# url-kaist/Quatro

Measured on AMD Instinct MI355X. Metric: scan-pair registrations/sec (KITTI 64-ch, ~5k corr) + rot/trans err vs ref, higher is better.
Workload: dtype f32 (voxel grid, FPFH, 33-D matching: f16-split MFMA filter, exact f32 decision) / f64 (consistency graph, GNC-TLS, COTE); 1 GPU; composite: qtr_register_pair_corr per step on a synthetic KITTI-64-shaped scan pair (voxel 0.3 m), back end on 5000 planted correspondences, one pair at a time, inputs resident in HBM (--full: the detailed description)

## Files before the change

quatro_amd/csrc/capi.hip:

```cpp
#include <dlfcn.h>

#include <algorithm>
#include <atomic>
#include <memory>
#include <mutex>
#include <new>
#include <thread>
#include <vector>

#include "common.h"
#include "frontend.h"
#include "solver.h"
#include "stage_times.h"

struct RcclIdByValue {
  char internal[QTR_COMM_ID_BYTES];
};

struct Slot {
  hipStream_t stream = nullptr;
  hipStream_t stream2 = nullptr;
  hipEvent_t ev[EV_COUNT] = {};
  hipEvent_t ev_vox = nullptr;
  hipStream_t stream3 = nullptr;
// ... 108 lines not shown
  int spin_wait = 1;
  bool pre_on = false;
  qtr_pw_params pre_pw;
  qtr_ip_params pre_ip;
  std::atomic<bool> long_lists{false};
  struct Callers {
    std::atomic<int> live{0};
  };
  std::shared_ptr<Callers> callers = std::make_shared<Callers>();
  std::mutex share_mu;
  int share_val = 1, share_gen = 0;
  std::atomic<int> gen_inflight[4] = {};
  unsigned long long uid = 0;
  int stage_events = 1;
  int corr_overlap = 1;
  int nn_event_stride = 1;
  int icp_block = 0;
  std::mutex kf_mu;
  std::vector<qtr_keyframe*> keyframes;
  std::vector<qtr_place_index*> place_indexes;
  std::vector<qtr_voxel_map*> voxel_maps;
  char err[512];
};

static std::atomic<unsigned long long> g_handle_uid{0};
static void vmap_free_all(qtr_handle* h);

#define QTR_TRY(expr)                  \
  do {                                 \
    const int rc_ = (expr);            \
// ... 368 lines not shown
  if (!out) return QTR_ERR_BAD_ARG;
  *out = nullptr;
  qtr_handle* h = new (std::nothrow) qtr_handle();
  if (!h) return QTR_ERR_CAPACITY;
  h->err[0] = 0;
  h->device = device;
  h->uid = g_handle_uid.fetch_add(1, std::memory_order_relaxed) + 1;
  {
    const char* hw = getenv("QTR_HOST_WAIT");
    h->spin_wait = (hw && strcmp(hw, "block") == 0) ? 0 : 1;
    const char* se = getenv("QTR_STAGE_EVENTS");
    h->stage_events = (se && atoi(se) == 0) ? 0 : 1;
    h->nn_event_stride = h->stage_events ? 1 : 0;
    const char* co = getenv("QTR_CORR_OVERLAP");
    h->corr_overlap = (co && atoi(co) == 0) ? 0 : 1;
    const char* ib = getenv("QTR_ICP_BLOCK");
    h->icp_block = ib ? std::max(0, atoi(ib)) : 0;
  }
  if (limits)
    h->lim = *limits;
  else
    qtr_default_limits(&h->lim);
  if (h->lim.max_points < 64 || h->lim.max_voxels < 64 || h->lim.max_corr < 64 || h->lim.n_slots < 1 ||
      h->lim.max_corr > 32768 || h->lim.max_voxels > h->lim.max_points || h->lim.max_long_neighbors < 0 ||
      h->lim.max_voxels > QTR_NN_MAX_ROWS) {
    delete h;
    return QTR_ERR_BAD_ARG;
  }
  if (h->lim.max_long_neighbors == 0)
    h->lim.max_long_neighbors = (int)std::min<long long>(128LL * h->lim.max_voxels, 1LL << 30);
// ... 1057 lines not shown
  int prio_least = 0, prio_greatest = 0;
  QTR_HIP_TRY(h, hipDeviceGetStreamPriorityRange(&prio_least, &prio_greatest));
  if (!s.ev_fork) QTR_HIP_TRY(h, hipEventCreateWithFlags(&s.ev_fork, hipEventDisableTiming));
  if (!s.ev_join) QTR_HIP_TRY(h, hipEventCreateWithFlags(&s.ev_join, hipEventDisableTiming));
  if (prio_greatest != prio_least) QTR_HIP_TRY(h, hipStreamCreateWithPriority(&s.stream3, hipStreamNonBlocking, prio_least));
  else QTR_HIP_TRY(h, hipStreamCreateWithFlags(&s.stream3, hipStreamNonBlocking));
  return QTR_OK;
}

struct CorrEarly {
  const float* src = nullptr;
  const float* tgt = nullptr;
  int n = 0, mem = QTR_MEM_HOST;
  const qtr_params* prm = nullptr;
  bool enqueued = false;
  int seq = 0;
  const float4 *cs = nullptr, *ct = nullptr;
  std::unique_ptr<InFlight> in_flight;
};
static int corr_early_enqueue(qtr_handle* h, Slot& s, CorrEarly& ce) {
  ce.enqueued = true;
  const bool ev_on = h->stage_events != 0;
  QTR_HIP_TRY(h, hipStreamWaitEvent(s.stream3, s.ev_fork, 0));
  if (ev_on) QTR_HIP_TRY(h, hipEventRecord(s.ev[EV_BE0], s.stream3));
  QTR_TRY(corr_stage(h, s, ce.src, ce.tgt, ce.n, ce.mem, s.stream3, &ce.cs, &ce.ct));
  s.last_L = ce.n;
  s.last_Wb = (((ce.n + 63) / 64) + 3) & ~3;
  s.sb.mail_seq = ce.seq = ++s.seq;
  ce.in_flight.reset(new InFlight(h));
  QTR_HIP_TRY(h, solver_enqueue(s.sb, ce.cs, ce.ct, ce.n, *ce.prm, s.stream3, ev_on ? s.ev[EV_GRAPH] : nullptr,
                                ev_on ? s.ev[EV_CLIQUE] : nullptr, false, true));
  if (ev_on) QTR_HIP_TRY(h, hipEventRecord(s.ev[EV_SOLVE], s.stream3));
  return QTR_OK;
}

struct CountsText {
  char s[40];
  CountsText(int nc, int a, int b, const char* pair_form = "%d / %d") { snprintf(s, sizeof(s), nc > 1 ? pair_form : "%d", a, b); }
// ... 68 lines not shown
  if (fp->normal_radius > fp->fpfh_radius) {
    snprintf(h->err, sizeof(h->err), "[FPFHManager]: Normal should be lower than fpfh_radius!!!!");
    return QTR_ERR_BAD_ARG;
  }
  if (Ps <= 0 || Pt <= 0 || !src_raw4 || !tgt_raw4) {
    snprintf(h->err, sizeof(h->err), "Invalid or empty point cloud dataset given!");
    return QTR_ERR_BAD_ARG;
  }
  if (Ps > h->lim.max_points || Pt > h->lim.max_points) {
    snprintf(h->err, sizeof(h->err), "cloud exceeds max_points=%d", h->lim.max_points);
    return QTR_ERR_CAPACITY;
  }
  QTR_HIP_TRY(h, hipSetDevice(h->device));
  if (early && !early->enqueued) {
    QTR_TRY(ensure_stream3(h, s));
    QTR_HIP_TRY(h, hipEventRecord(s.ev_fork, s.stream));
  }
  const float4 *d_s = (const float4*)src_raw4, *d_t = (const float4*)tgt_raw4;
  if (mem == QTR_MEM_HOST) {
    QTR_HIP_TRY(h, hipMemcpyAsync(s.in_src, src_raw4, (size_t)Ps * 16, hipMemcpyHostToDevice, s.stream));
    QTR_HIP_TRY(h, hipMemcpyAsync(s.in_tgt, tgt_raw4, (size_t)Pt * 16, hipMemcpyHostToDevice, s.stream));
    d_s = s.in_src;
    d_t = s.in_tgt;
  }
  if (h->stage_events) QTR_HIP_TRY(h, hipEventRecord(s.ev[EV_BEGIN], s.stream));
  const float4* raws[2] = {d_s, d_t};
  const int P2[2] = {Ps, Pt};
  auto beside_voxels = [&]() -> int {
    QTR_HIP_TRY(h, hipEventRecord(s.ev_vox, s.stream));
    const int on_device[2] = {-1, -1};
    QTR_HIP_TRY(h, hipStreamWaitEvent(s.stream2, s.ev_vox, 0));
// ... 70 lines not shown
    struct DrainOnReturn {
      hipStream_t st;
      bool armed = true;
      ~DrainOnReturn() {
        if (armed) (void)hipStreamSynchronize(st);
      }
    } drain{s.stream3};
    if (rc == QTR_OK) rc = wait_mail(h, s, s.stream3, MAIL_SEQ_SOLVE, ce.seq);
    if (rc == QTR_OK) rc = solve_followup(h, s, ce.cs, ce.ct, n_corr, prm, s.stream3, h->stage_events != 0);
    if (rc != QTR_OK) {
      return res->status = rc;
    }
    ce.in_flight.reset();
    result_from_mail(s, res);
    rc = res->status;
    QTR_HIP_TRY(h, hipEventRecord(s.ev_join, s.stream3));
    QTR_HIP_TRY(h, hipStreamWaitEvent(s.stream, s.ev_join, 0));
    if (h->stage_events) QTR_HIP_TRY(h, hipEventRecord(s.ev[EV_END], s.stream));
    rc = finish_registration(h, s, rc, TIMES_PAIR_OVERLAP, res, clique, nullptr, final_inliers, cap, mem_out, s.stream);
    drain.armed = rc != QTR_OK && rc != QTR_ERR_CLIQUE_TOO_SMALL;
    return rc;
  }
  int rc = front_device(h, s, src_raw4, Ps, tgt_raw4, Pt, fp, mem_in, true, &res->n_src, &res->n_tgt, &L, given);
  if (n_matched) *n_matched = L;
  res->n_corr = given ? n_corr : L;
  if (rc != QTR_OK) return res->status = rc;
  const float4 *cs = s.m_src, *ct = s.m_tgt;
  if (given) QTR_TRY(corr_stage(h, s, corr_src, corr_tgt, n_corr, mem_out, s.stream, &cs, &ct));
  rc = solve_device(h, s, cs, ct, res->n_corr, prm, res, true);
  return finish_registration(h, s, rc, TIMES_PAIR, res, clique, nullptr, final_inliers, cap, mem_out, s.stream);
}

// ... 2072 lines not shown
```

quatro_amd/csrc/frontend.h:

```cpp
#pragma once
#include "common.h"
#include "front_verdict.h"

#define QTR_KMAX 256
#define NBIG_LDS_KEYS 8192
#define RADIX_TILE 1024
#define NORM_BINS 192

#define QTR_NN_MAX_ROWS ((1 << 20) - 32)
#define QTR_CELL_CAP (1 << 21)
enum { MC_NCORR = 0, MC_HIDDEN_I = 1, MC_HIDDEN_J = 2, MC_NCROSS = 3, MC_NTUPLE = 4, MC_SWAPPED = 5, MC_NQ0 = 6, MC_NHIT = 7,
       MC_RECHECK0 = 8, MC_RECHECK1 = 9, MC_NSPLIT0 = 10, MC_NSPLIT1 = 11 ,
       MC_UNSAFE = 12,
       MC_TAILERR = 13  };

enum { MAIL_VOX0 = 0, MAIL_VOX1 = 16, MAIL_MATCH = 32, MAIL_CNT0 = 48, MAIL_CNT1 = 64, MAIL_SEQ_VOX0 = 96, MAIL_SEQ_VOX1 = 97,
       MAIL_SEQ_MATCH = 98, MAIL_SEQ_SOLVE = 99, MAIL_SEQ_ICP_BOX = 100, MAIL_SEQ_ICP = 101, MAIL_SOLVER = 128,
       MAIL_ICP_BOX = 256, MAIL_ICP = 272, MAIL_INTS = 512 };

struct CloudBufs {
  int* counts = nullptr;
  u32* mm = nullptr;
  u32* mm_part = nullptr;
  float4* vox = nullptr;
// ... 86 lines not shown
  const float* QT;
  int qt_pad;
  const float* baseTb;
  const int* brow;
  const int* bstart;
  const int* qorder;
  u64* best;
  int nq_slot, rc_slot;
};
struct NnPartial {
  float b1, b2;
  int i1;
  int pad;
};
#define TAIL_MAXWG 256
struct MatchView {
  NnDir d[2];
  const float4 *vox_i, *vox_j;
  const float *mean_i, *mean_j;
  const float *fpfh_i, *fpfh_j;
  float *baseT_i, *queryT_i, *norms_i, *baseT_j, *queryT_j, *norms_j;
  float *baseTb_i, *baseTb_j;
  uint4 *baseH_i, *baseH_j, *queryH_i, *queryH_j, *queryH_c;
  int *nb_row_i, *nb_row_j, *nb_start_i, *nb_start_j;
  u64 *hash_i, *hash_j, *table_i, *table_j;
  int dd_mask;
  int n_large, n_small, pad_large, pad_small, swapped, ns, nt;
  u64 *best_small, *best_large;
  int *nn_of_small, *nn_of_large, *cross_i, *cross_j, *flags, *scan, *passed, *tgt_of_src, *corr, *mcounts;
  NnPartial* partial;
// ... 45 lines not shown
  float* queryT_c = nullptr;
  float* norms_c = nullptr;
  uint4* queryH_c = nullptr;
  int dd_slots = 0;
  int *nc_cnt = nullptr, *nc_fill = nullptr, *nc_off = nullptr, *nc_list = nullptr;
  int* mail = nullptr;
  float4* m_src = nullptr;
  float4* m_tgt = nullptr;
  int m_cap = 0;
  int vox_passes = 4;
  int vox_fewer = 0;
  bool gathered = false;
  int mail_seq = 0;
  int nn_engine = 2;
  int n_cu = 256;
  int nn_events = 1;
  hipEvent_t ev_nn[4] = {};
};

size_t frontend_scratch_bytes(int max_points, int max_voxels);
void frontend_carve(FrontBufs& F, void* base, int max_points, int max_voxels);
hipError_t frontend_init_attributes();

hipError_t voxelize_enqueue(FrontBufs& F, int nc, const float4* const* raw, const int* P, float leaf, hipStream_t st,
                            int passes = 4, float cell_side = 0.f);
hipError_t set_count_enqueue(CloudBufs& C, int which, int value, hipStream_t st);
hipError_t fpfh_enqueue(FrontBufs& F, int first, int nc, const int* n, float r_normal, float r_fpfh, hipStream_t st,
                        bool with_mean, bool origin_known, bool long_lists, bool desc_prep = false,
                        int max_ncell = 0 );
hipError_t mean_enqueue(FrontBufs& F, int first, int nc, const int* n, hipStream_t st, int cap = 0);
// ... 16 lines not shown
```

quatro_amd/csrc/frontend.hip:

```cpp
#include <stdlib.h>

#include <type_traits>
#include <vector>

#include "common.h"
#include "frontend.h"

__device__ __forceinline__ u32 enc_f32(float f) {
  const u32 b = __float_as_uint(f);
  return (b & 0x80000000u) ? ~b : (b | 0x80000000u);
}
__device__ __forceinline__ float dec_f32(u32 e) {
  const u32 b = (e & 0x80000000u) ? (e & 0x7fffffffu) : ~e;
  return __uint_as_float(b);
}


__global__ void k_set_count(int* counts, int which, int value) {
  if (threadIdx.x == 0 && blockIdx.x == 0) counts[which] = value;
}

__device__ __forceinline__ void d_minmax(const float4* __restrict__ pts, int n, u32* __restrict__ part) {
  float mn[3] = {INFINITY, INFINITY, INFINITY}, mx[3] = {-INFINITY, -INFINITY, -INFINITY};
  for (int i = blockIdx.x * blockDim.x + threadIdx.x; i < n; i += gridDim.x * blockDim.x) {
// ... 1706 lines not shown
  while (m < 2 * max_voxels) m <<= 1;
  return m;
}
size_t frontend_scratch_bytes(int max_points, int max_voxels) {
  size_t per_cloud = 0;
  per_cloud += 4096 + MM_MAX_PARTS * 32 + 256;
  per_cloud += (size_t)max_voxels * (16 + 16 + 132 + 132);
  per_cloud += 2 * (size_t)max_points * 8;
  per_cloud += (size_t)(4096 * ((max_points + RADIX_TILE - 1) / RADIX_TILE) + 8192) * 4 + 65536;
  per_cloud += (size_t)((max_points + RADIX_TILE - 1) / RADIX_TILE + 64) * 4 * (RADIX_TILE / VOX_TILE_SINGLE) + 256;
  per_cloud += (size_t)max_voxels * 4 * 2 + 64;
  per_cloud += (size_t)max_voxels * QTR_KMAX * 8;
  per_cloud += (size_t)max_voxels * (16 + 72) + 512;
  per_cloud += 2 * (size_t)(QTR_CELL_CAP + 4096) * 4 + 512;
  per_cloud += (size_t)max_points * 16 + 256;
  size_t shared = (size_t)max_voxels * 64 + 16384 + 2 * TAIL_MAXWG * 4;
  shared += (size_t)max_voxels * (4 + 4 + 4 + 8) + (size_t)max_voxels * 4 * 6 + 4096;
  const size_t vpad = ((size_t)max_voxels + 511) / 512 * 512;
  per_cloud += 3 * 34 * vpad * 4 + (size_t)max_voxels * 8 + 4096;
  per_cloud += 2 * (vpad * 224 + 2 * 7168) + 512;
  per_cloud += (size_t)max_voxels * 8 + (size_t)dedup_slots(max_voxels) * 8 + 512;
  shared += vpad * 32 * 16 + 4 * ((size_t)max_voxels * 4 + 1024);
  shared += (size_t)max_voxels * 4 + 34 * vpad * 4 + vpad * 4 + 1024;
  shared += vpad * 224 + 2 * 7168 + 256 + (size_t)max_voxels * 4 + 1024;
  return 2 * per_cloud + shared + 64 * 256;
}

void frontend_carve(FrontBufs& F, void* base, int max_points, int max_voxels) {
  char* p = (char*)base;
  auto take = [&](size_t bytes) {
    char* r = p;
// ... 34 lines not shown
    C.nb_row = (int*)take((size_t)max_voxels * 4);
    C.nb_start = (int*)take((NORM_BINS + 2) * 4);
    C.norms = (float*)take((size_t)max_voxels * 4);
    C.max_norm = (u32*)take(64);
    C.dd_hash = (u64*)take((size_t)max_voxels * 8);
    C.dd_table = (u64*)take((size_t)dedup_slots(max_voxels) * 8);
  }
  F.dd_slots = dedup_slots(max_voxels);
  F.best_small = (u64*)take((size_t)max_voxels * 8);
  F.best_large = (u64*)take((size_t)max_voxels * 8);
  F.nn_of_small = (int*)take((size_t)max_voxels * 4);
  F.nn_of_large = (int*)take((size_t)max_voxels * 4);
  F.cross_i = (int*)take((size_t)max_voxels * 8);
  F.cross_j = (int*)take((size_t)max_voxels * 8);
  F.flags = (int*)take((size_t)max_voxels * 4);
  F.scan = (int*)take((size_t)max(max_voxels + 1, 2 * TAIL_MAXWG) * 4);
  F.passed = (int*)take((size_t)max_voxels * 8);
  F.tgt_of_src = (int*)take((size_t)max_voxels * 4);
  F.corr = (int*)take((size_t)max_voxels * 16);
  F.nc_cnt = (int*)take((size_t)max_voxels * 4);
  F.nc_fill = (int*)take((size_t)max_voxels * 4);
  F.nc_off = (int*)take((size_t)(max_voxels + 1) * 4);
  F.nc_list = (int*)take((size_t)max_voxels * 8);
  F.mcounts = (int*)take(16 * 4);
  F.nn_partial = take((((size_t)max_voxels + 511) / 512 * 512) * 32 * 16);
  F.recheck_rows = (int*)take((size_t)max_voxels * 4);
  F.recheck_thr = (float*)take((size_t)max_voxels * 4);
  F.recheck_span = (int2*)take((size_t)max_voxels * 8);
  F.hit_rows = (int*)take((size_t)max_voxels * 4);
  F.queryT_c = (float*)take(34 * (((size_t)max_voxels + 511) / 512 * 512) * 4);
  F.norms_c = (float*)take((((size_t)max_voxels + 511) / 512 * 512) * 4);
  F.queryH_c = (uint4*)take((((size_t)max_voxels + 511) / 512 * 512) * 224 + 2 * 7168);
  F.recheck_q = (int*)take((size_t)max_voxels * 4);
  {
    const char* e = QTR_ENGINE_ENV("QTR_NN_ENGINE");
    F.nn_engine = (e && strcmp(e, "exact") == 0) ? 0 : (e && strcmp(e, "mfma32") == 0) ? 1 : 2;
    int dev = 0, cus = 0;
    if (hipGetDevice(&dev) == hipSuccess &&
        hipDeviceGetAttribute(&cus, hipDeviceAttributeMultiprocessorCount, dev) == hipSuccess && cus > 0)
      F.n_cu = cus;
  }
}

hipError_t match_init_attributes();
hipError_t frontend_init_attributes() {
  hipError_t e;
  if ((e = hipFuncSetAttribute((const void*)k2_neighbors_big<false>, hipFuncAttributeMaxDynamicSharedMemorySize,
                               NBIG_LDS_KEYS * 8)) != hipSuccess)
    return e;
  if ((e = hipFuncSetAttribute((const void*)k2_neighbors_big<true>, hipFuncAttributeMaxDynamicSharedMemorySize,
                               NBIG_LDS_KEYS * 8)) != hipSuccess)
// ... 4 lines not shown
```

quatro_amd/csrc/match.hip:

```cpp
#include <vector>

#include "common.h"
#include "frontend.h"

#define NN_TILE 64
#define CROSS_LDS_BYTES (156 * 1024)
#define NN_STRIDE 36

#define LAUNCH_MV_K(kern, K, a, grid, block, lds, st, ...)                                                       \
  do {                                                                                                          \
    if ((a).ext)                                                                                                \
      hipLaunchKernelGGL((kern<true, K>), grid, block, lds, st, (ViewExt<MatchView>{(a).ext, {0, 0, 0}}), (a).one, ##__VA_ARGS__); \
    else                                                                                                        \
      hipLaunchKernelGGL((kern<false, K>), grid, block, lds, st, (ViewExt<MatchView>{nullptr, {0, 0, 0}}), (a).one, ##__VA_ARGS__); \
  } while (0)
#define LAUNCH_MV_EV(kern, a, grid, block, lds, st, e0, e1, ...)                                                 \
  do {                                                                                                          \
    if ((a).ext)                                                                                                \
      hipExtLaunchKernelGGL((kern<true>), grid, block, lds, st, e0, e1, 0, (ViewExt<MatchView>{(a).ext, {0, 0, 0}}), (a).one, ##__VA_ARGS__);  \
    else                                                                                                        \
      hipExtLaunchKernelGGL((kern<false>), grid, block, lds, st, e0, e1, 0, (ViewExt<MatchView>{nullptr, {0, 0, 0}}), (a).one, ##__VA_ARGS__); \
  } while (0)
#define LAUNCH_MV(kern, a, grid, block, lds, st, ...)                                       \
  do {                                                                                      \
// ... 1265 lines not shown
    for (int i = threadIdx.x; i < n_zero; i += blockDim.x) zero_words[i] = 0;
  if (gid < 16) V.mcounts[gid] = (gid == MC_SWAPPED) ? V.swapped : (gid == MC_NQ0) ? V.n_small : 0;
  const int pv = V.tuple ? 0 : 1;
  const int np = V.crosscheck ? V.n_small : V.n_small + V.n_large;
  for (int i = gid; i < np; i += gsz) V.passed[i] = pv;
  if (!V.crosscheck)
    for (int i = gid; i < V.ns; i += gsz) V.nc_cnt[i] = V.nc_fill[i] = 0;
  for (int i = gid; i < V.ns; i += gsz) V.tgt_of_src[i] = -1;
  for (int i = gid; i < V.n_small; i += gsz) V.best_small[i] = ~0ULL;
  for (int i = gid; i < V.n_large; i += gsz) V.best_large[i] = ~0ULL;
  if (clear_tables)
    for (int i = gid; i <= V.dd_mask; i += gsz) {
      V.table_i[i] = ~0ULL;
      V.table_j[i] = ~0ULL;
    }
  for (int i = gid; i < 2 * TAIL_MAXWG; i += gsz) V.scan[i] = 0;
}

template <bool EXT>
__global__ __launch_bounds__(1024) void k_hit_compact(ViewExt<MatchView> x, MatchView one, int bin_order, int nn_X) {
  const MatchView& V = EXT ? x.ext[blockIdx.z] : one;
  extern __shared__ u32 hit_bits[];
  __shared__ int wsum[16];
  const int tid = threadIdx.x, lane = tid & 63, wave = tid >> 6;
  const int n = V.n_large, nw = (n + 31) / 32, ns = V.n_small;
  QTR_STAMP(STAMP_HIT_COMPACT, 0)
  for (int w = tid; w < nw; w += 1024) hit_bits[w] = 0u;
  __syncthreads();
  for (int j0 = tid; j0 < ns; j0 += 16 * 1024) {
    u64 b[16];
#pragma unroll
// ... 99 lines not shown
    V.flags[i] = V.crosscheck ? ((b != ~0ULL && back == i) ? 1 : 0) : ((b != ~0ULL) ? 1 : 0);
  }
}

template <bool EXT>
__global__ __launch_bounds__(1024) void k_scan_flags(ViewExt<MatchView> x, MatchView one) {
  const MatchView& V = EXT ? x.ext[blockIdx.z] : one;
  d_block_scan(V.flags, V.scan, V.n_large, [](int x) { return x; });
}
template <bool EXT>
__global__ __launch_bounds__(1024) void k_scan_nonneg(ViewExt<MatchView> x, MatchView one) {
  const MatchView& V = EXT ? x.ext[blockIdx.z] : one;
  d_block_scan(V.tgt_of_src, V.scan, V.ns, [](int x) { return x >= 0 ? 1 : 0; });
}

__device__ __forceinline__ void match_mail(const MatchView& V, int t, int total, int ntuple) {
  int* mail = V.mail;
  if (t < 16)
    mail_store_line(mail + MAIL_MATCH, t, (t == MC_NCORR) ? total : (t == MC_NTUPLE) ? ntuple : V.mcounts[t], V.seq);
  else if (t < 32)
    mail_store_line(mail + MAIL_CNT0, t - 16, V.counts0[t - 16], V.seq);
  else
    mail_store_line(mail + MAIL_CNT1, t - 32, V.counts1[t - 32], V.seq);
  __threadfence_system();
  if (t == 0) mail[MAIL_SEQ_MATCH] = V.seq;
}

template <bool EXT>
__global__ void k_corr_compact2(ViewExt<MatchView> x, MatchView one) {
  const MatchView& V = EXT ? x.ext[blockIdx.z] : one;
  const int ns = V.ns;
  for (int s = blockIdx.x * blockDim.x + threadIdx.x; s < ns; s += gridDim.x * blockDim.x) {
    const int t = V.tgt_of_src[s];
    if (t >= 0) {
// ... 3 lines not shown
  }
  if (blockIdx.x == 0 && threadIdx.x == 0) V.mcounts[MC_NCORR] = V.scan[ns];
  if (V.mail && blockIdx.x == 0 && threadIdx.x < 48) match_mail(V, threadIdx.x, V.scan[ns], V.mcounts[MC_NTUPLE]);
}

template <bool EXT>
__global__ void k_cross_compact(ViewExt<MatchView> x, MatchView one) {
  const MatchView& V = EXT ? x.ext[blockIdx.z] : one;
  for (int i = blockIdx.x * blockDim.x + threadIdx.x; i < V.n_large; i += gridDim.x * blockDim.x) {
    if (V.flags[i]) {
      V.cross_i[V.scan[i]] = i;
      V.cross_j[V.scan[i]] = V.nn_of_large[i];
    }
  }
  if (blockIdx.x == 0 && threadIdx.x == 0) V.mcounts[MC_NCROSS] = V.scan[V.n_large];
}

template <bool EXT>
__global__ __launch_bounds__(256) void k_tuple(ViewExt<MatchView> x, MatchView one) {
  const MatchView& V = EXT ? x.ext[blockIdx.z] : one;
  if (!V.tuple) return;
  const int ncorr = V.mcounts[MC_NCROSS];
  if (ncorr <= 0) return;
  const float4* __restrict__ pts_i = V.vox_i;
  const float4* __restrict__ pts_j = V.vox_j;
  const int* __restrict__ cross_i = V.cross_i;
  const int* __restrict__ cross_j = V.cross_j;
  const float scale = V.tuple_scale;
  const u64 seed = V.seed;
  const long long trials = (long long)ncorr * 100;
  const float mix = V.mean_i[0], miy = V.mean_i[1], miz = V.mean_i[2];
  const float mjx = V.mean_j[0], mjy = V.mean_j[1], mjz = V.mean_j[2];
  for (long long t = (long long)blockIdx.x * blockDim.x + threadIdx.x; t < trials;
       t += (long long)gridDim.x * blockDim.x) {
    const int r0 = (int)(qm_rand_u32(seed, 3ULL * (u64)t) % (u32)ncorr);
    const int r1 = (int)(qm_rand_u32(seed, 3ULL * (u64)t + 1ULL) % (u32)ncorr);
    const int r2 = (int)(qm_rand_u32(seed, 3ULL * (u64)t + 2ULL) % (u32)ncorr);
    float pi[3][3], pj[3][3];
    const int rr[3] = {r0, r1, r2};
#pragma unroll
    for (int k = 0; k < 3; ++k) {
      const float4 pa = pts_i[cross_i[rr[k]]], pb = pts_j[cross_j[rr[k]]];
      pi[k][0] = pa.x - mix;
      pi[k][1] = pa.y - miy;
      pi[k][2] = pa.z - miz;
      pj[k][0] = pb.x - mjx;
      pj[k][1] = pb.y - mjy;
      pj[k][2] = pb.z - mjz;
    }
    float li[3], lj[3];
#pragma unroll
    for (int k = 0; k < 3; ++k) {
      const int k2 = (k + 1) % 3;
      float dx = pi[k][0] - pi[k2][0], dy = pi[k][1] - pi[k2][1], dz = pi[k][2] - pi[k2][2];
      li[k] = sqrtf(dx * dx + (dy * dy + dz * dz));
      dx = pj[k][0] - pj[k2][0];
      dy = pj[k][1] - pj[k2][1];
      dz = pj[k][2] - pj[k2][2];
      lj[k] = sqrtf(dx * dx + (dy * dy + dz * dz));
    }
    if ((li[0] * scale < lj[0]) && (lj[0] < li[0] / scale) && (li[1] * scale < lj[1]) && (lj[1] < li[1] / scale) &&
        (li[2] * scale < lj[2]) && (lj[2] < li[2] / scale)) {
      V.passed[r0] = 1;
      V.passed[r1] = 1;
      V.passed[r2] = 1;
    }
  }
}

template <bool EXT>
__global__ void k_scatter_pairs(ViewExt<MatchView> x, MatchView one) {
  const MatchView& V = EXT ? x.ext[blockIdx.z] : one;
  const int nc = V.mcounts[MC_NCROSS];
  const int swapped = V.swapped;
  int local = 0;
  for (int c = blockIdx.x * blockDim.x + threadIdx.x; c < nc; c += gridDim.x * blockDim.x) {
    if (V.passed[c]) {
// ... 457 lines not shown
    if (tt[k] >= 0) {
      const int src = s0 + 2 * tid + k;
      V.corr[2 * run] = src;
      V.corr[2 * run + 1] = tt[k];
      if (V.m_src && run < V.m_cap) {
        float4 pa = V.vox_s[src], pb = V.vox_t[tt[k]];
        pa.w = 0.f;
        pb.w = 0.f;
        V.m_src[run] = pa;
        V.m_tgt[run] = pb;
      }
      ++run;
    }
}

__global__ void k_gather_matched(const float4* __restrict__ vs, const float4* __restrict__ vt,
                                 const int* __restrict__ corr, int L, float4* __restrict__ ms, float4* __restrict__ mt) {
  for (int c = blockIdx.x * blockDim.x + threadIdx.x; c < L; c += gridDim.x * blockDim.x) {
    float4 a = vs[corr[2 * c]], b = vt[corr[2 * c + 1]];
    a.w = 0.f;
    b.w = 0.f;
    ms[c] = a;
    mt[c] = b;
  }
}

static_assert(CM_ROWS == 512 && PM_SRC == 512, "TAIL_MAXWG look-back words cover TAIL_MAXWG * 512 rows");
static bool tail_is_fused(bool crosscheck, int max_large, int max_ns) {
  static const bool tail_single = [] {
    const char* e = QTR_ENGINE_ENV("QTR_MATCH_TAIL");
    return e && strcmp(e, "single") == 0;
  }();
  const int lim = tail_single ? 32768 : TAIL_MAXWG * 512;
  return crosscheck && max_large <= lim && max_ns <= lim;
}
static inline int grid_for(int n) {
  int g = (n + 255) / 256;
  return g < 1 ? 1 : (g > 2048 ? 2048 : g);
}

static MatchView make_match_view(FrontBufs& F, int ns, int nt, const qtr_frontend_params& fp, unsigned long long seed) {
  MatchView V;
  memset(&V, 0, sizeof(V));
  const int swapped = nt > ns ? 1 : 0;
  CloudBufs& Ci = F.cloud[swapped ? 1 : 0];
  CloudBufs& Cj = F.cloud[swapped ? 0 : 1];
  V.swapped = swapped;
  V.ns = ns;
// ... 100 lines not shown
  d1.qmap = F.hit_rows;
  d1.nq_pad = V.pad_large;
  d1.A = Ci.fpfh;
  d1.QT = Ci.queryT;
  d1.qt_pad = V.pad_large;
  d1.baseTb = Cj.baseTb;
  d1.brow = Cj.nb_row;
  d1.bstart = Cj.nb_start;
  d1.qorder = nullptr;
  d1.best = F.best_large;
  d1.nq_slot = MC_NHIT;
  d1.rc_slot = MC_RECHECK1;
  return V;
}

static hipError_t match_launch(const MatchView* views, int G, int nn_engine, int n_cu, ViewStage* stage,
                               hipStream_t st, hipEvent_t const* ev, bool init_done = false, bool prep_done = false) {
  MatchArgs a;
  a.one = views[0];
  a.ext = nullptr;
  if (G > 1) {
    a.ext = (const MatchView*)stage_push(stage, views, sizeof(MatchView) * (size_t)G, st);
    if (!a.ext) return hipErrorOutOfMemory;
  }
  int max_large = 1, max_small = 1, max_ns = 1, max_pad = NN_QPB;
  bool any_tuple = false;
  for (int g = 0; g < G; ++g) {
    max_large = max(max_large, views[g].n_large);
    max_small = max(max_small, views[g].n_small);
    max_ns = max(max_ns, views[g].ns);
    max_pad = max(max_pad, views[g].pad_large);
    any_tuple = any_tuple || views[g].tuple;
// ... 84 lines not shown
      if (!f16) LAUNCH_MV(k_nn_exact_rows, a, dim3(ex, ey, G), B256, 0, st, dir);
#else
      (void)ex;
      (void)ey;
#endif
    };
    run_dir(0, max_small, max_large, ev ? ev[0] : nullptr, ev ? ev[1] : nullptr);
    LAUNCH_MV(k_hit_compact, a, dim3(1, 1, G), dim3(1024), (size_t)((max_large + 31) / 32) * 4, st, f16 ? 0 : 1,
              (f16 && G == 1) ? X : 0);
#ifdef QTR_TEST_ENGINES
    if (!f16) LAUNCH_MV(k_hit_gather, a, dim3(max_pad / 256, 1, G), B256, 0, st, 1);
#endif
    run_dir(1, max_large, max_small, ev ? ev[2] : nullptr, ev ? ev[3] : nullptr);
  }
  const bool crosscheck = views[0].crosscheck != 0;
  const bool fused_tail = tail_is_fused(crosscheck, max_large, max_ns);
  const bool fused16 = max_large <= 16384 && max_ns <= 16384;
  static const bool tail_single = [] {
    const char* e = QTR_ENGINE_ENV("QTR_MATCH_TAIL");
    return e && strcmp(e, "single") == 0;
  }();
  const bool tail_multi = fused_tail && !tail_single;
  if (!crosscheck) {
    LAUNCH_MV(k_cross_flags2, a, dim3(grid_for(max_large), 1, G), B256, 0, st);
    LAUNCH_MV(k_scan_flags, a, dim3(1, 1, G), dim3(1024), 0, st);
    LAUNCH_MV(k_nc_list, a, dim3(grid_for(max_large + max_small), 1, G), B256, 0, st);
  } else if (fused_tail) {
    const int lds_gather = ((size_t)max_large + (size_t)max_small) * 4 <= (size_t)CROSS_LDS_BYTES ? 1 : 0;
    const size_t cross_lds = (size_t)max_large * 4 + (lds_gather ? (size_t)max_small * 4 : 0);
    if (tail_multi) LAUNCH_MV(k_cross_multi, a, dim3((max_large + CM_ROWS - 1) / CM_ROWS, 1, G), B256, 0, st);
#ifdef QTR_TEST_ENGINES
    else if (fused16) LAUNCH_MV_K(k_cross_fused, 16, a, dim3(1, 1, G), dim3(1024), cross_lds, st, lds_gather);
    else LAUNCH_MV_K(k_cross_fused, 32, a, dim3(1, 1, G), dim3(1024), cross_lds, st, lds_gather);
#else
    (void)cross_lds;
    (void)fused16;
#endif
// ... 27 lines not shown

hipError_t match_init_enqueue(FrontBufs& F, int ns, int nt, const qtr_frontend_params& fp, hipStream_t st, bool clear_tables,
                              int* zero_words, int n_zero) {
  (void)hipGetLastError();
  MatchArgs a;
  a.one = make_match_view(F, ns, nt, fp, (unsigned long long)fp.seed);
  a.ext = nullptr;
  LAUNCH_MV(k_match_init, a, dim3(grid_for(max(a.one.n_large, a.one.dd_mask + 1)), 1, 1), dim3(256), 0, st, clear_tables ? 1 : 0, zero_words, n_zero);
  return hipGetLastError();
}
hipError_t match_enqueue(FrontBufs& F, int ns, int nt, const qtr_frontend_params& fp, hipStream_t st, bool init_done,
                         bool prep_done, bool gather) {
  (void)hipGetLastError();
  MatchView V = make_match_view(F, ns, nt, fp, (unsigned long long)fp.seed);
  if (!gather) V.m_src = V.m_tgt = nullptr;
  const bool fused_tail = tail_is_fused(V.crosscheck != 0, V.n_large, ns);
  F.gathered = fused_tail && V.m_src != nullptr;
  const bool evs = F.nn_events != 0;
  return match_launch(&V, 1, F.nn_engine, F.n_cu, nullptr, st, evs ? F.ev_nn : nullptr, init_done, prep_done);
}

hipError_t match_enqueue_group(FrontBufs* const* F, int G, const int* n, const qtr_frontend_params* fp,
                               const unsigned long long* seeds, ViewStage* stage, hipStream_t st, bool prep_done) {
  (void)hipGetLastError();
  std::vector<MatchView> v((size_t)G);
  int max_large = 1, max_ns = 1;
  for (int g = 0; g < G; ++g) {
    v[g] = make_match_view(*F[g], n[2 * g], n[2 * g + 1], *fp, seeds[g]);
    max_large = max(max_large, v[g].n_large);
    max_ns = max(max_ns, v[g].ns);
  }
  const bool fused_tail = tail_is_fused(fp->use_crosscheck != 0, max_large, max_ns);
  for (int g = 0; g < G; ++g) F[g]->gathered = fused_tail && F[g]->m_src != nullptr;
  return match_launch(v.data(), G, F[0]->nn_engine, F[0]->n_cu, stage, st, nullptr, false, prep_done);
}

hipError_t gather_matched_enqueue(FrontBufs& F, int L, float4* m_src, float4* m_tgt, hipStream_t st) {
  if (L <= 0 || (F.gathered && m_src == F.m_src && m_tgt == F.m_tgt)) return hipSuccess;
  hipLaunchKernelGGL(k_gather_matched, dim3(grid_for(L)), dim3(256), 0, st, F.cloud[0].vox, F.cloud[1].vox, F.corr, L,
                     m_src, m_tgt);
  return hipGetLastError();
}

hipError_t match_init_attributes() {
  hipError_t e;
  (void)e;
#ifdef QTR_TEST_ENGINES
  if ((e = hipFuncSetAttribute((const void*)k_cross_fused<false, 16>, hipFuncAttributeMaxDynamicSharedMemorySize, CROSS_LDS_BYTES)) != hipSuccess) return e;
  if ((e = hipFuncSetAttribute((const void*)k_cross_fused<true, 16>, hipFuncAttributeMaxDynamicSharedMemorySize, CROSS_LDS_BYTES)) != hipSuccess) return e;
  if ((e = hipFuncSetAttribute((const void*)k_cross_fused<false, 32>, hipFuncAttributeMaxDynamicSharedMemorySize, CROSS_LDS_BYTES)) != hipSuccess) return e;
  if ((e = hipFuncSetAttribute((const void*)k_cross_fused<true, 32>, hipFuncAttributeMaxDynamicSharedMemorySize, CROSS_LDS_BYTES)) != hipSuccess) return e;
#define SET_LDS2(kern)                                                                                                   \
  if ((e = hipFuncSetAttribute((const void*)kern<false, 32>, hipFuncAttributeMaxDynamicSharedMemorySize, 132 * 1024)) != hipSuccess) \
    return e;                                                                                                            \
  if ((e = hipFuncSetAttribute((const void*)kern<true, 32>, hipFuncAttributeMaxDynamicSharedMemorySize, 132 * 1024)) != hipSuccess)  \
    return e;
  SET_LDS2(k_pairs_fused)
#undef SET_LDS2
#endif
  return hipSuccess;
}
// ... 1 lines not shown
```

Baseline: 2862 registrations/s.

## Fuse cross-check, tuple test and compaction into one multi-block match tail kernel

Adds k_match_tail, which combines cross-check gathering, the tuple consistency trials and the final compaction into one launch with a last-block ticket. By default (TAIL_TWO) it runs after k_cross_multi for single-view matching. This replaces a sequence of tail kernels and is meant to cut launch count and inter-kernel gaps. Separately, the fork event is skipped when the main stream is already idle, and when no outputs or stage events are needed the join event is replaced by a host synchronize. This trades event overhead for a blocking wait and adds a global atomic ticket that must be reset on each run.

Result: no change. 2858 registrations/s (-0.1%).

```diff
diff --git a/quatro_amd/csrc/capi.hip b/quatro_amd/csrc/capi.hip
--- a/quatro_amd/csrc/capi.hip
+++ b/quatro_amd/csrc/capi.hip
@@ -146,6 +146,7 @@
   unsigned long long uid = 0;
   int stage_events = 1;
   int corr_overlap = 1;
+  bool fork_always = false, join_always = false;
   int nn_event_stride = 1;
   int icp_block = 0;
   std::mutex kf_mu;
@@ -544,6 +545,9 @@
     h->nn_event_stride = h->stage_events ? 1 : 0;
     const char* co = getenv("QTR_CORR_OVERLAP");
     h->corr_overlap = (co && atoi(co) == 0) ? 0 : 1;
+    const char* pm = QTR_ENGINE_ENV("QTR_PAIR_MARKERS");
+    h->fork_always = pm && (strcmp(pm, "fork") == 0 || strcmp(pm, "both") == 0);
+    h->join_always = pm && (strcmp(pm, "join") == 0 || strcmp(pm, "both") == 0);
     const char* ib = getenv("QTR_ICP_BLOCK");
     h->icp_block = ib ? std::max(0, atoi(ib)) : 0;
   }
@@ -1631,6 +1635,7 @@
   int n = 0, mem = QTR_MEM_HOST;
   const qtr_params* prm = nullptr;
   bool enqueued = false;
+  bool forked = false;
   int seq = 0;
   const float4 *cs = nullptr, *ct = nullptr;
   std::unique_ptr<InFlight> in_flight;
@@ -1638,7 +1643,7 @@
 static int corr_early_enqueue(qtr_handle* h, Slot& s, CorrEarly& ce) {
   ce.enqueued = true;
   const bool ev_on = h->stage_events != 0;
-  QTR_HIP_TRY(h, hipStreamWaitEvent(s.stream3, s.ev_fork, 0));
+  if (ce.forked) QTR_HIP_TRY(h, hipStreamWaitEvent(s.stream3, s.ev_fork, 0));
   if (ev_on) QTR_HIP_TRY(h, hipEventRecord(s.ev[EV_BE0], s.stream3));
   QTR_TRY(corr_stage(h, s, ce.src, ce.tgt, ce.n, ce.mem, s.stream3, &ce.cs, &ce.ct));
   s.last_L = ce.n;
@@ -1737,7 +1742,11 @@
   QTR_HIP_TRY(h, hipSetDevice(h->device));
   if (early && !early->enqueued) {
     QTR_TRY(ensure_stream3(h, s));
-    QTR_HIP_TRY(h, hipEventRecord(s.ev_fork, s.stream));
+    const hipError_t q = h->fork_always ? hipErrorNotReady : hipStreamQuery(s.stream);
+    if (q != hipSuccess && q != hipErrorNotReady) QTR_HIP_TRY(h, q);
+    (void)hipGetLastError();
+    early->forked = q != hipSuccess;
+    if (early->forked) QTR_HIP_TRY(h, hipEventRecord(s.ev_fork, s.stream));
   }
   const float4 *d_s = (const float4*)src_raw4, *d_t = (const float4*)tgt_raw4;
   if (mem == QTR_MEM_HOST) {
@@ -1838,8 +1847,12 @@
     ce.in_flight.reset();
     result_from_mail(s, res);
     rc = res->status;
-    QTR_HIP_TRY(h, hipEventRecord(s.ev_join, s.stream3));
-    QTR_HIP_TRY(h, hipStreamWaitEvent(s.stream, s.ev_join, 0));
+    if (clique || final_inliers || h->stage_events || h->join_always) {
+      QTR_HIP_TRY(h, hipEventRecord(s.ev_join, s.stream3));
+      QTR_HIP_TRY(h, hipStreamWaitEvent(s.stream, s.ev_join, 0));
+    } else {
+      QTR_HIP_TRY(h, hipStreamSynchronize(s.stream3));
+    }
     if (h->stage_events) QTR_HIP_TRY(h, hipEventRecord(s.ev[EV_END], s.stream));
     rc = finish_registration(h, s, rc, TIMES_PAIR_OVERLAP, res, clique, nullptr, final_inliers, cap, mem_out, s.stream);
     drain.armed = rc != QTR_OK && rc != QTR_ERR_CLIQUE_TOO_SMALL;
diff --git a/quatro_amd/csrc/frontend.h b/quatro_amd/csrc/frontend.h
--- a/quatro_amd/csrc/frontend.h
+++ b/quatro_amd/csrc/frontend.h
@@ -124,6 +124,8 @@
   int pad;
 };
 #define TAIL_MAXWG 256
+enum { TAIL_ONE = 0, TAIL_MULTI = 1, TAIL_SINGLE = 2, TAIL_TWO = 3 };
+#define TAIL_ONE_WGS 256
 struct MatchView {
   NnDir d[2];
   const float4 *vox_i, *vox_j;
@@ -199,6 +201,8 @@
   int mail_seq = 0;
   int nn_engine = 2;
   int n_cu = 256;
+  int match_tail = TAIL_TWO;
+  int tail_wgs = TAIL_ONE_WGS;
   int nn_events = 1;
   hipEvent_t ev_nn[4] = {};
 };
diff --git a/quatro_amd/csrc/frontend.hip b/quatro_amd/csrc/frontend.hip
--- a/quatro_amd/csrc/frontend.hip
+++ b/quatro_amd/csrc/frontend.hip
@@ -1744,7 +1744,7 @@
   per_cloud += (size_t)max_voxels * (16 + 72) + 512;
   per_cloud += 2 * (size_t)(QTR_CELL_CAP + 4096) * 4 + 512;
   per_cloud += (size_t)max_points * 16 + 256;
-  size_t shared = (size_t)max_voxels * 64 + 16384 + 2 * TAIL_MAXWG * 4;
+  size_t shared = (size_t)max_voxels * 64 + 16384 + 2 * TAIL_MAXWG * 4 + 256;
   shared += (size_t)max_voxels * (4 + 4 + 4 + 8) + (size_t)max_voxels * 4 * 6 + 4096;
   const size_t vpad = ((size_t)max_voxels + 511) / 512 * 512;
   per_cloud += 3 * 34 * vpad * 4 + (size_t)max_voxels * 8 + 4096;
@@ -1809,7 +1809,7 @@
   F.cross_i = (int*)take((size_t)max_voxels * 8);
   F.cross_j = (int*)take((size_t)max_voxels * 8);
   F.flags = (int*)take((size_t)max_voxels * 4);
-  F.scan = (int*)take((size_t)max(max_voxels + 1, 2 * TAIL_MAXWG) * 4);
+  F.scan = (int*)take((size_t)max(max_voxels + 1, 2 * TAIL_MAXWG + 1) * 4);
   F.passed = (int*)take((size_t)max_voxels * 8);
   F.tgt_of_src = (int*)take((size_t)max_voxels * 4);
   F.corr = (int*)take((size_t)max_voxels * 16);
@@ -1830,6 +1830,10 @@
   {
     const char* e = QTR_ENGINE_ENV("QTR_NN_ENGINE");
     F.nn_engine = (e && strcmp(e, "exact") == 0) ? 0 : (e && strcmp(e, "mfma32") == 0) ? 1 : 2;
+    const char* t = QTR_ENGINE_ENV("QTR_MATCH_TAIL");
+    F.match_tail = (t && strcmp(t, "single") == 0) ? TAIL_SINGLE : (t && strcmp(t, "multi") == 0) ? TAIL_MULTI : (t && strcmp(t, "one") == 0) ? TAIL_ONE : TAIL_TWO;
+    const char* tw = QTR_ENGINE_ENV("QTR_MATCH_TAIL_WGS");
+    if (tw && atoi(tw) >= 1 && atoi(tw) <= 1024) F.tail_wgs = atoi(tw);
     int dev = 0, cus = 0;
     if (hipGetDevice(&dev) == hipSuccess &&
         hipDeviceGetAttribute(&cus, hipDeviceAttributeMultiprocessorCount, dev) == hipSuccess && cus > 0)
diff --git a/quatro_amd/csrc/match.hip b/quatro_amd/csrc/match.hip
--- a/quatro_amd/csrc/match.hip
+++ b/quatro_amd/csrc/match.hip
@@ -1303,7 +1303,7 @@
       V.table_i[i] = ~0ULL;
       V.table_j[i] = ~0ULL;
     }
-  for (int i = gid; i < 2 * TAIL_MAXWG; i += gsz) V.scan[i] = 0;
+  for (int i = gid; i < 2 * TAIL_MAXWG + 1; i += gsz) V.scan[i] = 0;
 }
 
 template <bool EXT>
@@ -1433,10 +1433,12 @@
   d_block_scan(V.tgt_of_src, V.scan, V.ns, [](int x) { return x >= 0 ? 1 : 0; });
 }
 
-__device__ __forceinline__ void match_mail(const MatchView& V, int t, int total, int ntuple) {
+__device__ __forceinline__ void match_mail(const MatchView& V, int t, int total, int ntuple, int ncross = -1) {
   int* mail = V.mail;
   if (t < 16)
-    mail_store_line(mail + MAIL_MATCH, t, (t == MC_NCORR) ? total : (t == MC_NTUPLE) ? ntuple : V.mcounts[t], V.seq);
+    mail_store_line(mail + MAIL_MATCH, t,
+                    (t == MC_NCORR) ? total : (t == MC_NTUPLE) ? ntuple : (t == MC_NCROSS && ncross >= 0) ? ncross : V.mcounts[t],
+                    V.seq);
   else if (t < 32)
     mail_store_line(mail + MAIL_CNT0, t - 16, V.counts0[t - 16], V.seq);
   else
@@ -1470,6 +1472,33 @@
     }
   }
   if (blockIdx.x == 0 && threadIdx.x == 0) V.mcounts[MC_NCROSS] = V.scan[V.n_large];
+}
+
+__device__ __forceinline__ bool tuple_trial_ok(const float4 (&pa)[3], const float4 (&pb)[3], float mix, float miy, float miz,
+                                               float mjx, float mjy, float mjz, float scale) {
+  float pi[3][3], pj[3][3];
+#pragma unroll
+  for (int k = 0; k < 3; ++k) {
+    pi[k][0] = pa[k].x - mix;
+    pi[k][1] = pa[k].y - miy;
+    pi[k][2] = pa[k].z - miz;
+    pj[k][0] = pb[k].x - mjx;
+    pj[k][1] = pb[k].y - mjy;
+    pj[k][2] = pb[k].z - mjz;
+  }
+  float li[3], lj[3];
+#pragma unroll
+  for (int k = 0; k < 3; ++k) {
+    const int k2 = (k + 1) % 3;
+    float dx = pi[k][0] - pi[k2][0], dy = pi[k][1] - pi[k2][1], dz = pi[k][2] - pi[k2][2];
+    li[k] = sqrtf(dx * dx + (dy * dy + dz * dz));
+    dx = pj[k][0] - pj[k2][0];
+    dy = pj[k][1] - pj[k2][1];
+    dz = pj[k][2] - pj[k2][2];
+    lj[k] = sqrtf(dx * dx + (dy * dy + dz * dz));
+  }
+  return (li[0] * scale < lj[0]) && (lj[0] < li[0] / scale) && (li[1] * scale < lj[1]) && (lj[1] < li[1] / scale) &&
+         (li[2] * scale < lj[2]) && (lj[2] < li[2] / scale);
 }
 
 template <bool EXT>
@@ -1492,31 +1521,14 @@
     const int r0 = (int)(qm_rand_u32(seed, 3ULL * (u64)t) % (u32)ncorr);
     const int r1 = (int)(qm_rand_u32(seed, 3ULL * (u64)t + 1ULL) % (u32)ncorr);
     const int r2 = (int)(qm_rand_u32(seed, 3ULL * (u64)t + 2ULL) % (u32)ncorr);
-    float pi[3][3], pj[3][3];
     const int rr[3] = {r0, r1, r2};
+    float4 pa[3], pb[3];
 #pragma unroll
     for (int k = 0; k < 3; ++k) {
-      const float4 pa = pts_i[cross_i[rr[k]]], pb = pts_j[cross_j[rr[k]]];
-      pi[k][0] = pa.x - mix;
-      pi[k][1] = pa.y - miy;
-      pi[k][2] = pa.z - miz;
-      pj[k][0] = pb.x - mjx;
-      pj[k][1] = pb.y - mjy;
-      pj[k][2] = pb.z - mjz;
-    }
-    float li[3], lj[3];
-#pragma unroll
-    for (int k = 0; k < 3; ++k) {
-      const int k2 = (k + 1) % 3;
-      float dx = pi[k][0] - pi[k2][0], dy = pi[k][1] - pi[k2][1], dz = pi[k][2] - pi[k2][2];
-      li[k] = sqrtf(dx * dx + (dy * dy + dz * dz));
-      dx = pj[k][0] - pj[k2][0];
-      dy = pj[k][1] - pj[k2][1];
-      dz = pj[k][2] - pj[k2][2];
-      lj[k] = sqrtf(dx * dx + (dy * dy + dz * dz));
-    }
-    if ((li[0] * scale < lj[0]) && (lj[0] < li[0] / scale) && (li[1] * scale < lj[1]) && (lj[1] < li[1] / scale) &&
-        (li[2] * scale < lj[2]) && (lj[2] < li[2] / scale)) {
+      pa[k] = pts_i[cross_i[rr[k]]];
+      pb[k] = pts_j[cross_j[rr[k]]];
+    }
+    if (tuple_trial_ok(pa, pb, mix, miy, miz, mjx, mjy, mjz, scale)) {
       V.passed[r0] = 1;
       V.passed[r1] = 1;
       V.passed[r2] = 1;
@@ -2004,6 +2016,207 @@
     }
 }
 
+#define MT_MAX_ROWS 32768
+#define MT_KMAX (MT_MAX_ROWS / 1024)
+#define MT_BIT_WORDS (MT_MAX_ROWS / 32)
+#define MT_LDS_BYTES(n_small) (((size_t)(n_small) + 2 * MT_BIT_WORDS) * 4)
+__global__ __launch_bounds__(1024) void k_match_tail(MatchView V, int from_global) {
+  extern __shared__ u32 mt_s[];
+  __shared__ int wsum[16];
+  __shared__ int s_ticket, s_ntuple;
+  const int tid = threadIdx.x, lane = tid & 63, wave = tid >> 6;
+  const int n_large = V.n_large, n_small = V.n_small;
+  const int W = gridDim.x, w = blockIdx.x;
+  u32* list = mt_s;
+  u32* bits = mt_s + (from_global ? 0 : n_small);
+  u32* pre = bits + MT_BIT_WORDS;
+  QTR_STAMP(STAMP_CROSS, 0)
+  int nc = 0;
+  if (!from_global) {
+  const u32* __restrict__ lo_small = (const u32*)V.best_small;
+  const u32* __restrict__ lo_large = (const u32*)V.best_large;
+  const int K = (n_large + 1023) >> 10, row0 = wave * 64 * K + lane;
+  const int per = (n_small + W - 1) / W, m0 = w * per, m1 = min(n_small, m0 + per);
+  u32 bs[16];
+  int jj[MT_KMAX];
+#pragma unroll
+  for (int q = 0; q < 16; ++q) bs[q] = (tid + q * 1024 < n_small) ? lo_small[2u * (u32)(tid + q * 1024)] : ~0u;
+#pragma unroll
+  for (int k = 0; k < MT_KMAX; ++k) {
+    const int i = row0 + k * 64;
+    jj[k] = (k < K && i < n_large) ? (int)lo_large[2u * (u32)i] : -1;
+  }
+#pragma unroll
+  for (int q = 0; q < 16; ++q) {
+    const int j = tid + q * 1024;
+    if (j < n_small) {
+      const int v = (bs[q] == ~0u) ? 0 : (int)bs[q];
+      list[j] = (u32)v;
+      if (j >= m0 && j < m1) V.nn_of_small[j] = v;
+    }
+  }
+  for (int j = tid + 16 * 1024; j < n_small; j += 1024) {
+    const u32 b = lo_small[2u * (u32)j];
+    const int v = (b == ~0u) ? 0 : (int)b;
+    list[j] = (u32)v;
+    if (j >= m0 && j < m1) V.nn_of_small[j] = v;
+  }
+  __syncthreads();
+  u32 keep = 0;
+#pragma unroll
+  for (int k = 0; k < MT_KMAX; ++k) {
+    if (k < K) {
+      const int i = row0 + k * 64;
+      const bool asked = jj[k] != -1;
+      const int j = asked ? jj[k] : 0;
+      const int back = (j < n_small) ? (int)list[j] : -1;
+      jj[k] = j;
+      if (asked && back == i) keep |= 1u << k;
+      if (w == 0 && i < n_large) V.nn_of_large[i] = asked ? j : -1;
+    }
+  }
+  {
+    const int wt = wave_sum_i32(__popc(keep));
+    if (lane == 0) wsum[wave] = wt;
+  }
+  __syncthreads();
+  int run = 0;
+#pragma unroll
+  for (int q = 0; q < 16; ++q) {
+    run += (q < wave) ? wsum[q] : 0;
+    nc += wsum[q];
+  }
+#pragma unroll
+  for (int k = 0; k < MT_KMAX; ++k) {
+    if (k < K) {
+      const bool kp = ((keep >> k) & 1u) != 0;
+      const u64 m = __ballot(kp);
+      if (kp) {
+        const int r = run + __popcll(m & lanemask_lt()), i = row0 + k * 64;
+        list[r] = ((u32)i << 16) | (u32)jj[k];
+        if (w == 0) {
+          V.cross_i[r] = i;
+          V.cross_j[r] = jj[k];
+        }
+      }
+      run += __popcll(m);
+    }
+  }
+  if (w == 0 && tid == 0) V.mcounts[MC_NCROSS] = nc;
+  __syncthreads();
+  } else {
+    nc = V.mcounts[MC_NCROSS];
+  }
+  const int* __restrict__ g_ci = V.cross_i;
+  const int* __restrict__ g_cj = V.cross_j;
+  auto entry = [&](int r) -> u32 { return from_global ? (((u32)g_ci[r] << 16) | (u32)g_cj[r]) : list[r]; };
+  QTR_STAMP(STAMP_CROSS, 1)
+  if (V.tuple && nc > 0) {
+    const float4* __restrict__ pts_i = V.vox_i;
+    const float4* __restrict__ pts_j = V.vox_j;
+    const float scale = V.tuple_scale;
+    const u64 seed = V.seed;
+    const long long trials = (long long)nc * 100;
+    const float mix = V.mean_i[0], miy = V.mean_i[1], miz = V.mean_i[2];
+    const float mjx = V.mean_j[0], mjy = V.mean_j[1], mjz = V.mean_j[2];
+    for (long long t = (long long)w * 1024 + tid; t < trials; t += (long long)W * 1024) {
+      const int r0 = (int)(qm_rand_u32(seed, 3ULL * (u64)t) % (u32)nc);
+      const int r1 = (int)(qm_rand_u32(seed, 3ULL * (u64)t + 1ULL) % (u32)nc);
+      const int r2 = (int)(qm_rand_u32(seed, 3ULL * (u64)t + 2ULL) % (u32)nc);
+      const int rr[3] = {r0, r1, r2};
+      float4 pa[3], pb[3];
+#pragma unroll
+      for (int k = 0; k < 3; ++k) {
+        const u32 e = entry(rr[k]);
+        pa[k] = pts_i[e >> 16];
+        pb[k] = pts_j[e & 0xffffu];
+      }
+      if (tuple_trial_ok(pa, pb, mix, miy, miz, mjx, mjy, mjz, scale)) {
+        V.passed[r0] = 1;
+        V.passed[r1] = 1;
+        V.passed[r2] = 1;
+      }
+    }
+  }
+  asm volatile("s_waitcnt vmcnt(0)" ::: "memory");
+  __syncthreads();
+  QTR_STAMP(STAMP_CROSS, 2)
+  if (tid == 0) s_ticket = __hip_atomic_fetch_add(V.scan + 2 * TAIL_MAXWG, 1, __ATOMIC_ACQ_REL, __HIP_MEMORY_SCOPE_AGENT);
+  __syncthreads();
+  QTR_STAMP(STAMP_CROSS, 3)
+  if (s_ticket != W - 1) return;
+  const int swapped = V.swapped;
+  bits[tid] = 0u;
+  if (tid == 0) s_ntuple = 0;
+  __syncthreads();
+  u32 pm = 0;
+  int local = 0;
+  for (int k0 = 0; k0 * 1024 < nc; k0 += 8) {
+    int pf[8];
+#pragma unroll
+    for (int q = 0; q < 8; ++q) {
+      const int c = tid + (k0 + q) * 1024;
+      pf[q] = (c < nc) ? __hip_atomic_load(V.passed + c, __ATOMIC_RELAXED, __HIP_MEMORY_SCOPE_AGENT) : 0;
+    }
+#pragma unroll
+    for (int q = 0; q < 8; ++q)
+      if (pf[q]) {
+        const u32 e = entry(tid + (k0 + q) * 1024);
+        const u32 src = swapped ? (e & 0xffffu) : (e >> 16);
+        atomicOr(&bits[src >> 5], 1u << (src & 31));
+        pm |= 1u << (k0 + q);
+        ++local;
+      }
+  }
+  QTR_STAMP(STAMP_CROSS, 4)
+  local = wave_sum_i32(local);
+  if (lane == 0 && local) atomicAdd(&s_ntuple, local);
+  __syncthreads();
+  int tot;
+  const int ex = wave_excl_scan_i32(__popc(bits[tid]), &tot);
+  if (lane == 63) wsum[wave] = tot;
+  __syncthreads();
+  int before = ex, total = 0;
+#pragma unroll
+  for (int q = 0; q < 16; ++q) {
+    before += (q < wave) ? wsum[q] : 0;
+    total += wsum[q];
+  }
+  pre[tid] = (u32)before;
+  __syncthreads();
+  const int ntuple = s_ntuple;
+  const bool tail_err = from_global && V.mcounts[MC_TAILERR] != 0;
+  if (V.mail && tid < 48) match_mail(V, tid, tail_err ? -1 : total, ntuple, nc);
+  if (tail_err) {
+    if (tid == 0) {
+      V.mcounts[MC_NCORR] = -1;
+      V.mcounts[MC_NTUPLE] = ntuple;
+    }
+    return;
+  }
+  for (int c = tid, k = 0; c < nc; c += 1024, ++k)
+    if ((pm >> k) & 1u) {
+      const u32 e = entry(c);
+      const int i = (int)(e >> 16), j = (int)(e & 0xffffu);
+      const int src = swapped ? j : i, tgt = swapped ? i : j;
+      const int r = (int)pre[src >> 5] + __popc(bits[src >> 5] & ((1u << (src & 31)) - 1u));
+      V.corr[2 * r] = src;
+      V.corr[2 * r + 1] = tgt;
+      if (V.m_src && r < V.m_cap) {
+        float4 pa = V.vox_s[src], pb = V.vox_t[tgt];
+        pa.w = 0.f;
+        pb.w = 0.f;
+        V.m_src[r] = pa;
+        V.m_tgt[r] = pb;
+      }
+    }
+  if (tid == 0) {
+    V.mcounts[MC_NCORR] = total;
+    V.mcounts[MC_NTUPLE] = ntuple;
+  }
+  QTR_STAMP(STAMP_CROSS, 5)
+}
+
 __global__ void k_gather_matched(const float4* __restrict__ vs, const float4* __restrict__ vt,
                                  const int* __restrict__ corr, int L, float4* __restrict__ ms, float4* __restrict__ mt) {
   for (int c = blockIdx.x * blockDim.x + threadIdx.x; c < L; c += gridDim.x * blockDim.x) {
@@ -2016,12 +2229,8 @@
 }
 
 static_assert(CM_ROWS == 512 && PM_SRC == 512, "TAIL_MAXWG look-back words cover TAIL_MAXWG * 512 rows");
-static bool tail_is_fused(bool crosscheck, int max_large, int max_ns) {
-  static const bool tail_single = [] {
-    const char* e = QTR_ENGINE_ENV("QTR_MATCH_TAIL");
-    return e && strcmp(e, "single") == 0;
-  }();
-  const int lim = tail_single ? 32768 : TAIL_MAXWG * 512;
+static bool tail_is_fused(bool crosscheck, int max_large, int max_ns, int tail_mode) {
+  const int lim = tail_mode == TAIL_SINGLE ? 32768 : TAIL_MAXWG * 512;
   return crosscheck && max_large <= lim && max_ns <= lim;
 }
 static inline int grid_for(int n) {
@@ -2152,8 +2361,9 @@
   return V;
 }
 
-static hipError_t match_launch(const MatchView* views, int G, int nn_engine, int n_cu, ViewStage* stage,
-                               hipStream_t st, hipEvent_t const* ev, bool init_done = false, bool prep_done = false) {
+static hipError_t match_launch(const MatchView* views, int G, int nn_engine, int n_cu, int tail_mode, int tail_wgs,
+                               ViewStage* stage, hipStream_t st, hipEvent_t const* ev, bool init_done = false,
+                               bool prep_done = false) {
   MatchArgs a;
   a.one = views[0];
   a.ext = nullptr;
@@ -2268,13 +2478,15 @@
     run_dir(1, max_large, max_small, ev ? ev[2] : nullptr, ev ? ev[3] : nullptr);
   }
   const bool crosscheck = views[0].crosscheck != 0;
-  const bool fused_tail = tail_is_fused(crosscheck, max_large, max_ns);
+  const bool fused_tail = tail_is_fused(crosscheck, max_large, max_ns, tail_mode);
   const bool fused16 = max_large <= 16384 && max_ns <= 16384;
-  static const bool tail_single = [] {
-    const char* e = QTR_ENGINE_ENV("QTR_MATCH_TAIL");
-    return e && strcmp(e, "single") == 0;
-  }();
-  const bool tail_multi = fused_tail && !tail_single;
+  const bool tail_multi = fused_tail && tail_mode != TAIL_SINGLE;
+  if (tail_multi && (tail_mode == TAIL_ONE || tail_mode == TAIL_TWO) && G == 1 && max_large <= MT_MAX_ROWS) {
+    const int two = tail_mode == TAIL_TWO ? 1 : 0;
+    if (two) LAUNCH_MV(k_cross_multi, a, dim3((max_large + CM_ROWS - 1) / CM_ROWS, 1, 1), B256, 0, st);
+    hipLaunchKernelGGL(k_match_tail, dim3(max(1, tail_wgs)), dim3(1024), MT_LDS_BYTES(two ? 0 : views[0].n_small), st, a.one, two);
+    return hipGetLastError();
+  }
   if (!crosscheck) {
     LAUNCH_MV(k_cross_flags2, a, dim3(grid_for(max_large), 1, G), B256, 0, st);
     LAUNCH_MV(k_scan_flags, a, dim3(1, 1, G), dim3(1024), 0, st);
@@ -2332,10 +2544,11 @@
   (void)hipGetLastError();
   MatchView V = make_match_view(F, ns, nt, fp, (unsigned long long)fp.seed);
   if (!gather) V.m_src = V.m_tgt = nullptr;
-  const bool fused_tail = tail_is_fused(V.crosscheck != 0, V.n_large, ns);
+  const bool fused_tail = tail_is_fused(V.crosscheck != 0, V.n_large, ns, F.match_tail);
   F.gathered = fused_tail && V.m_src != nullptr;
   const bool evs = F.nn_events != 0;
-  return match_launch(&V, 1, F.nn_engine, F.n_cu, nullptr, st, evs ? F.ev_nn : nullptr, init_done, prep_done);
+  return match_launch(&V, 1, F.nn_engine, F.n_cu, F.match_tail, F.tail_wgs, nullptr, st, evs ? F.ev_nn : nullptr, init_done,
+                      prep_done);
 }
 
 hipError_t match_enqueue_group(FrontBufs* const* F, int G, const int* n, const qtr_frontend_params* fp,
@@ -2348,9 +2561,10 @@
     max_large = max(max_large, v[g].n_large);
     max_ns = max(max_ns, v[g].ns);
   }
-  const bool fused_tail = tail_is_fused(fp->use_crosscheck != 0, max_large, max_ns);
+  const bool fused_tail = tail_is_fused(fp->use_crosscheck != 0, max_large, max_ns, F[0]->match_tail);
   for (int g = 0; g < G; ++g) F[g]->gathered = fused_tail && F[g]->m_src != nullptr;
-  return match_launch(v.data(), G, F[0]->nn_engine, F[0]->n_cu, stage, st, nullptr, false, prep_done);
+  return match_launch(v.data(), G, F[0]->nn_engine, F[0]->n_cu, F[0]->match_tail, F[0]->tail_wgs, stage, st, nullptr, false,
+                      prep_done);
 }
 
 hipError_t gather_matched_enqueue(FrontBufs& F, int L, float4* m_src, float4* m_tgt, hipStream_t st) {
@@ -2362,7 +2576,7 @@
 
 hipError_t match_init_attributes() {
   hipError_t e;
-  (void)e;
+  if ((e = hipFuncSetAttribute((const void*)k_match_tail, hipFuncAttributeMaxDynamicSharedMemorySize, (int)MT_LDS_BYTES(MT_MAX_ROWS))) != hipSuccess) return e;
 #ifdef QTR_TEST_ENGINES
   if ((e = hipFuncSetAttribute((const void*)k_cross_fused<false, 16>, hipFuncAttributeMaxDynamicSharedMemorySize, CROSS_LDS_BYTES)) != hipSuccess) return e;
   if ((e = hipFuncSetAttribute((const void*)k_cross_fused<true, 16>, hipFuncAttributeMaxDynamicSharedMemorySize, CROSS_LDS_BYTES)) != hipSuccess) return e;
```
